# Sleepwalking/libllsm2

Hardware: AMD Instinct MI355X
Metric: frames/sec (layer0 analyze+synth, 44.1 kHz, 5 ms hop) (higher is better)
Workload: dtype f32; 1 GPU; 1024 synthetic 1 s utterances per GPU, F0 120 Hz fixed, 44.1 kHz, 5 ms hop, layer0 analyze+synth, default options, f0_refine=0; utterances_per_gpu=1024, frames_per_utterance=200, parallelism=dp1

## Files before the change

include/llsm_gpu.h:

```cpp
#ifndef LLSM_AMD_LLSM_GPU_H
#define LLSM_AMD_LLSM_GPU_H

#include <stddef.h>
#include "llsm.h"

#ifdef __cplusplus
extern "C" {
#endif

typedef struct llsm_gpu_context llsm_gpu_context;
typedef struct llsm_gpu_batch   llsm_gpu_batch;

int         llsm_gpu_device_count(void);
const char* llsm_gpu_last_error(void);

llsm_gpu_context* llsm_gpu_create_context(int device, void* stream);
void              llsm_gpu_delete_context(llsm_gpu_context* ctx);
void*             llsm_gpu_context_stream(llsm_gpu_context* ctx);
int               llsm_gpu_synchronize(llsm_gpu_context* ctx);

int llsm_gpu_set_convention(const char* name, int value);
int llsm_gpu_get_convention(const char* name);

void llsm_gpu_release_cached_memory(void);
// ... 197 lines not shown
  FP_TYPE* eenv_ampl; FP_TYPE* eenv_phse;
} llsm_flat_params;
int llsm_chunk_to_flat(llsm_chunk* src, llsm_flat_params* dst, int frm_off);
void llsm_slab_stats(long long* live_slabs, long long* live_bytes, long long* pooled_bytes);
void llsm_slab_trim(void);
void llsm_delete_chunks(llsm_chunk** chunks, int n);
void llsm_gpu_release_cached_batches(void);
int llsm_flat_to_chunk(const llsm_flat_params* src, int frm_off, llsm_chunk* dst);

size_t      llsm_chunk_blob_size(llsm_chunk* src);
long long   llsm_chunk_to_blob(llsm_chunk* src, void* dst, size_t capacity);
int         llsm_blob_view(const void* blob, size_t bytes, llsm_flat_params* view, int* nfrm,
  FP_TYPE* thop, FP_TYPE* fnyq);
llsm_chunk* llsm_blob_to_chunk(const void* blob, size_t bytes);
int         llsm_blob_view_l1(const void* blob, size_t bytes, llsm_flat_l1* view);
int         llsm_gpu_batch_upload_blob(llsm_gpu_batch* b, int utt, const void* blob, size_t bytes);
int         llsm_gpu_batch_upload_blobs(llsm_gpu_batch* b, int utt0, int n, const void* const* blobs, const size_t* bytes);
size_t      llsm_blob_bytes(int nfrm, int maxnhar, int maxnhar_e, int npsd, int nchannel, int nchanfreq, int nspec);
int         llsm_gpu_batch_blob_sizes(llsm_gpu_batch* b, int utt0, int n, size_t* sizes);
int         llsm_gpu_batch_download_blobs(llsm_gpu_batch* b, int utt0, int n, void* const* dst, const size_t* capacity);
int         llsm_gpu_batch_download_blob_block(llsm_gpu_batch* b, int utt0, int n, void* block, size_t capacity, size_t* offsets);

typedef void llsm_rtsynth_group;
llsm_rtsynth_group* llsm_create_rtsynth_group(llsm_soptions* options, llsm_container* conf,
  int capacity_samples, int n_streams);
void llsm_delete_rtsynth_group(llsm_rtsynth_group* g);
int  llsm_rtsynth_group_getlatency(llsm_rtsynth_group* g);
int  llsm_rtsynth_group_numoutput(llsm_rtsynth_group* g, int stream);
void llsm_rtsynth_group_feed(llsm_rtsynth_group* g, llsm_container** frames);
void llsm_rtsynth_group_feed_many(llsm_rtsynth_group* g, llsm_container** frames, int n_hops);
int       llsm_gpu_rt_graph(int on);
int       llsm_gpu_shared_f0_tiles(int on);
int       llsm_gpu_synth_tables(int on);
int       llsm_gpu_pbp_real_ifft(int on);
int       llsm_gpu_analysis_overlap(int on);
long long llsm_gpu_rt_graph_hops(void);
int       llsm_gpu_rt_pipeline(int on);
int       llsm_gpu_rt_fused(int on);
int       llsm_gpu_rt_direct(int on);
int  llsm_rtsynth_group_fetch(llsm_rtsynth_group* g, int stream, FP_TYPE* dst_p, FP_TYPE* dst_ap,
  int max_samples);
int  llsm_rtsynth_group_fetch_all(llsm_rtsynth_group* g, FP_TYPE* dst_p, FP_TYPE* dst_ap, int max_samples,
  int* counts);

void llsm_gpu_set_default_seed(unsigned long long seed);

int llsm_gpu_plan_index(int which, int i, int j, FP_TYPE f0, FP_TYPE thop,
  FP_TYPE fs, FP_TYPE rel_winsize);

#ifdef __cplusplus
}
#endif
#endif
```

libllsm2_amd/__init__.py:

```python
import ctypes as C
import os

import numpy as np

_HERE = os.path.dirname(os.path.abspath(__file__))
LIB_PATH = os.environ.get("LLSM_AMD_LIB", os.path.join(_HERE, "libllsm2_amd.so"))

fp = C.c_float
P_fp = C.POINTER(C.c_float)
P_int = C.POINTER(C.c_int)


class Container(C.Structure):
    _fields_ = [("members", C.POINTER(C.c_void_p)), ("destructors", C.POINTER(C.c_void_p)),
                ("copyctors", C.POINTER(C.c_void_p)), ("nmember", C.c_int)]


class HMFrame(C.Structure):
    _fields_ = [("ampl", P_fp), ("phse", P_fp), ("nhar", C.c_int)]


class NMFrame(C.Structure):
    _fields_ = [("eenv", C.POINTER(C.POINTER(HMFrame))), ("edc", P_fp), ("psd", P_fp),
                ("npsd", C.c_int), ("nchannel", C.c_int)]
# ... 81 lines not shown
llsm_create_nmframe llsm_copy_nmframe llsm_copy_nmframe_inplace llsm_delete_nmframe
llsm_create_pbpeffect llsm_copy_pbpeffect llsm_delete_pbpeffect
llsm_create_frame llsm_frame_phaseshift llsm_frame_phasesync_rps llsm_frame_checklayer0
llsm_frame_checklayer1 llsm_conf_checklayer0 llsm_conf_checklayer1 llsm_delete_output
llsm_frame_tolayer0 llsm_chunk_tolayer1 llsm_chunk_tolayer0
llsm_gpu_batch_enable_layer1 llsm_gpu_batch_tolayer1 llsm_gpu_batch_tolayer0 llsm_gpu_batch_set_maxnhar_conf
llsm_gpu_batch_set_pbpeffect llsm_chunk_to_flat_l1 llsm_flat_l1_to_chunk
llsm_refine_f0 llsm_compute_spectrogram llsm_compute_dc llsm_harmonic_peakpicking llsm_harmonic_czt
llsm_harmonic_analysis llsm_subband_energy llsm_fft_to_psd llsm_estimate_psd llsm_warp_frequency
llsm_spectral_mean llsm_spectrum_from_envelope llsm_get_fftsize llsm_synthesize_harmonic_frame
llsm_synthesize_harmonic_frame_iczt llsm_generate_white_noise llsm_generate_bandlimited_noise
llsm_lipfilter llsm_lipfilter_reim llsm_harmonic_spectrum llsm_harmonic_envelope llsm_harmonic_minphase
llsm_create_cached_glottal_model llsm_delete_cached_glottal_model llsm_spectral_glottal_fitting
llsm_smoothing_filter llsm_lfmodel_from_rd llsm_lfmodel_spectrum llsm_lfmodel_to_gfm llsm_gfm_to_lfmodel
llsm_synthesize_harmonic_frame_auto llsm_make_filtered_pulse
llsm_create_coder llsm_delete_coder llsm_coder_encode llsm_coder_decode_layer1 llsm_coder_decode_layer0
llsm_coder_dimension llsm_coder_encode_frames llsm_coder_decode_frames
llsm_create_aoptions llsm_delete_aoptions llsm_aoptions_toconf
llsm_create_soptions llsm_delete_soptions
llsm_create_chunk llsm_copy_chunk llsm_delete_chunk llsm_chunk_phasesync_rps
llsm_chunk_phasepropagate llsm_chunk_getf0 llsm_analyze llsm_synthesize
llsm_create_rtsynth_buffer llsm_delete_rtsynth_buffer llsm_rtsynth_buffer_getlatency
llsm_rtsynth_buffer_numoutput llsm_rtsynth_buffer_feed llsm_rtsynth_buffer_fetch
llsm_rtsynth_buffer_fetch_decomposed llsm_rtsynth_buffer_clear
llsm_gpu_device_count llsm_gpu_last_error llsm_gpu_create_context llsm_gpu_delete_context
llsm_gpu_context_stream llsm_gpu_synchronize llsm_gpu_set_profiling llsm_gpu_profile_only llsm_gpu_reset_profile
llsm_gpu_get_profile llsm_gpu_fft_selftest llsm_gpu_release_cached_memory llsm_gpu_create_batch llsm_gpu_delete_batch llsm_gpu_batch_layout
llsm_gpu_batch_offsets llsm_gpu_alloc_host llsm_gpu_free_host llsm_gpu_batch_upload llsm_gpu_batch_download llsm_gpu_batch_device_ptr
llsm_gpu_batch_array_bytes llsm_gpu_batch_analyze llsm_gpu_batch_synthesize
llsm_analyze_batch llsm_synthesize_batch llsm_chunk_to_flat llsm_flat_to_chunk
llsm_gpu_set_default_seed llsm_gpu_plan_index llsm_gpu_batch_set_fnyq llsm_gpu_batch_debug_plane llsm_gpu_sum_outputs llsm_gpu_set_convention llsm_gpu_get_convention llsm_gpu_set_fanout llsm_fanout_plan llsm_fanout_selftest
llsm_chunk_blob_size llsm_chunk_to_blob llsm_blob_view llsm_blob_to_chunk llsm_blob_view_l1 llsm_gpu_batch_upload_blob llsm_gpu_batch_upload_blobs
llsm_create_rtsynth_group llsm_delete_rtsynth_group llsm_rtsynth_group_getlatency
llsm_rtsynth_group_numoutput llsm_rtsynth_group_feed llsm_rtsynth_group_feed_many llsm_rtsynth_group_fetch llsm_rtsynth_group_fetch_all llsm_gpu_rt_graph llsm_gpu_rt_graph_hops llsm_gpu_rt_fused llsm_gpu_rt_direct llsm_gpu_rt_pipeline llsm_gpu_analysis_overlap llsm_slab_stats llsm_slab_trim llsm_delete_chunks llsm_gpu_release_cached_batches llsm_gpu_device_numa_node llsm_gpu_bind_thread_to_device llsm_gpu_batch_packed_words llsm_gpu_batch_download_packed llsm_gpu_batch_upload_packed llsm_gpu_batch_download_outputs llsm_gpu_batch_download_packed_block llsm_gpu_batch_upload_packed_block llsm_gpu_batch_transfer_many llsm_gpu_batch_params_layout llsm_gpu_batch_transfer_params llsm_gpu_shared_f0_tiles llsm_gpu_synth_tables llsm_gpu_pbp_real_ifft llsm_frame_compute_snr
llsm_gpu_batch_phasesync_rps llsm_gpu_batch_phasepropagate llsm_gpu_batch_retime llsm_gpu_retime_uniform_positions
llsm_gpu_batch_pitch_formant llsm_gpu_batch_splice
llsm_gpu_batch_enable_coder llsm_gpu_batch_coder_dimension llsm_gpu_batch_encode llsm_gpu_batch_decode
llsm_blob_bytes llsm_gpu_batch_blob_sizes llsm_gpu_batch_download_blobs llsm_gpu_batch_download_blob_block
llsm_gpu_f0_default_options llsm_gpu_f0_plan llsm_gpu_batch_estimate_f0
llsm_gpu_f0_track_default_options llsm_gpu_f0_track_check llsm_gpu_batch_track_f0
llsm_gpu_align_default_options llsm_gpu_align_check llsm_gpu_batch_align
llsm_gpu_batch_align_band llsm_gpu_align_band_min llsm_gpu_align_band_rows
llsm_gpu_batch_align_slope llsm_gpu_align_slope_rows
llsm_gpu_batch_align_band_slope llsm_gpu_align_band_slope_min llsm_gpu_align_band_slope_rows
llsm_gpu_select_default_options llsm_gpu_select_check llsm_gpu_batch_select llsm_gpu_batch_select_chain
""".split()

_lib = None


def load():
    global _lib
    if _lib is not None:
        return _lib
    if not os.path.exists(LIB_PATH):
        from . import build as _b
        _b.build()
    L = C.CDLL(LIB_PATH)
    vp = C.c_void_p
    L.llsm_gpu_last_error.restype = C.c_char_p
    L.llsm_gpu_create_context.restype = vp
    L.llsm_gpu_create_context.argtypes = [C.c_int, vp]
    L.llsm_gpu_delete_context.argtypes = [vp]
    L.llsm_gpu_context_stream.restype = vp
    L.llsm_gpu_context_stream.argtypes = [vp]
    L.llsm_gpu_synchronize.argtypes = [vp]
    L.llsm_gpu_set_profiling.argtypes = [vp, C.c_int]
# ... 164 lines not shown
    L.llsm_copy_hmframe.restype = C.POINTER(HMFrame)
    L.llsm_copy_hmframe.argtypes = [C.POINTER(HMFrame)]
    L.llsm_delete_hmframe.argtypes = [C.POINTER(HMFrame)]
    L.llsm_hmframe_phaseshift.argtypes = [C.POINTER(HMFrame), fp]
    L.llsm_create_nmframe.restype = C.POINTER(NMFrame)
    L.llsm_create_nmframe.argtypes = [C.c_int, C.c_int, C.c_int]
    L.llsm_copy_nmframe.restype = C.POINTER(NMFrame)
    L.llsm_copy_nmframe.argtypes = [C.POINTER(NMFrame)]
    L.llsm_delete_nmframe.argtypes = [C.POINTER(NMFrame)]
    L.llsm_create_frame.restype = C.POINTER(Container)
    L.llsm_create_frame.argtypes = [C.c_int, C.c_int, C.c_int, C.c_int]
    L.llsm_frame_checklayer0.argtypes = [C.POINTER(Container)]
    L.llsm_conf_checklayer0.argtypes = [C.POINTER(Container)]
    L.llsm_create_rtsynth_buffer.restype = vp
    L.llsm_create_rtsynth_buffer.argtypes = [C.POINTER(SOptions), C.POINTER(Container), C.c_int]
    L.llsm_delete_rtsynth_buffer.argtypes = [vp]
    L.llsm_rtsynth_buffer_getlatency.argtypes = [vp]
    L.llsm_rtsynth_buffer_numoutput.argtypes = [vp]
    L.llsm_rtsynth_buffer_feed.argtypes = [vp, C.POINTER(Container)]
    L.llsm_rtsynth_buffer_fetch.argtypes = [vp, P_fp]
    L.llsm_rtsynth_buffer_fetch_decomposed.argtypes = [vp, P_fp, P_fp]
    L.llsm_rtsynth_buffer_clear.argtypes = [vp]
    L.llsm_create_rtsynth_group.restype = vp
    L.llsm_create_rtsynth_group.argtypes = [C.POINTER(SOptions), C.POINTER(Container), C.c_int, C.c_int]
    L.llsm_delete_rtsynth_group.argtypes = [vp]
    L.llsm_rtsynth_group_getlatency.argtypes = [vp]
    L.llsm_rtsynth_group_numoutput.argtypes = [vp, C.c_int]
    L.llsm_rtsynth_group_feed.argtypes = [vp, C.POINTER(C.POINTER(Container))]
    L.llsm_rtsynth_group_fetch.argtypes = [vp, C.c_int, P_fp, P_fp, C.c_int]
    L.llsm_rtsynth_group_fetch_all.argtypes = [vp, P_fp, P_fp, C.c_int, P_int]
    L.llsm_gpu_rt_graph.argtypes = [C.c_int]
    L.llsm_gpu_shared_f0_tiles.argtypes = [C.c_int]
    L.llsm_gpu_synth_tables.argtypes = [C.c_int]
    L.llsm_gpu_pbp_real_ifft.argtypes = [C.c_int]
    L.llsm_gpu_rt_fused.argtypes = [C.c_int]
    L.llsm_gpu_rt_direct.argtypes = [C.c_int]
    L.llsm_gpu_rt_pipeline.argtypes = [C.c_int]
    L.llsm_gpu_analysis_overlap.argtypes = [C.c_int]
    L.llsm_gpu_rt_graph_hops.restype = C.c_longlong
    _lib = L
    return L


class LlsmError(RuntimeError):
    pass


def _check(rc, what):
    if rc != 0:
        raise LlsmError(f"{what}: {load().llsm_gpu_last_error().decode()}")


def make_aoptions(**kw):
    o = AOptions()
    o.thop, o.maxnhar, o.maxnhar_e, o.npsd, o.nchannel = 0.005, 100, 4, 256, 4
    o.lip_radius, o.f0_refine, o.hm_method, o.rel_winsize = 1.5, 1, HMCZT, 4.0
    cf = kw.pop("chanfreq", [2000.0, 4000.0, 8000.0])
    for k, v in kw.items():
        setattr(o, k, v)
    o._cf = (fp * max(len(cf), 1))(*cf)
    o.chanfreq = C.cast(o._cf, P_fp)
    return o


def retime_uniform_positions(nfrm_src, nfrm_dst):
    pos = np.zeros(max(int(nfrm_dst), 0), np.float32)
# ... 423 lines not shown
```

libllsm2_amd/csrc/dev_common.h:

```cpp
#pragma once
#include <hip/hip_runtime.h>
#include <stdint.h>
#include "kernels.h"

#define WAVE 64
#define DEV __device__ __forceinline__

DEV float wave_sum(float v) {
#pragma unroll
  for(int o = 32; o > 0; o >>= 1) v += __shfl_xor(v, o, WAVE);
  return v;
}

DEV float wave_max(float v) {
#pragma unroll
  for(int o = 32; o > 0; o >>= 1) v = fmaxf(v, __shfl_xor(v, o, WAVE));
  return v;
}

typedef __amdgpu_buffer_rsrc_t buf_t;
DEV buf_t buf_range(const float* p, int lo, int hi) {
  const int n = hi > lo ? hi - lo : 0;
  return __builtin_amdgcn_make_buffer_rsrc((void*)(p + lo), 0, n * 4, 0x00020000);
}
DEV float ld_range(buf_t r, int idx_minus_lo) {
  int off = idx_minus_lo * 4;
  asm volatile("" : "+v"(off));
  return __builtin_bit_cast(float, __builtin_amdgcn_raw_buffer_load_b32(r, off, 0, 0));
}
DEV float ld_range_b(buf_t r, int byte_off) {
  asm volatile("" : "+v"(byte_off));
  return __builtin_bit_cast(float, __builtin_amdgcn_raw_buffer_load_b32(r, byte_off, 0, 0));
}

DEV void cs_turns(double turns, float* c, float* s) {
  const float y = (float)((turns - rint(turns)) * 4.0);
  const float k = rintf(y);
  const float r = y - k, r2 = r * r;
  float sn = fmaf(r2, 1.6044118478735982e-4f, -4.681754135318688e-3f);
  sn = fmaf(r2, sn, 7.969262624616704e-2f);
  sn = fmaf(r2, sn, -6.459640975062462e-1f);
  sn = fmaf(r2, sn, 1.5707963267948966f) * r;
  float cs = fmaf(r2, -2.5202042373060605e-5f, 9.1926027483942658e-4f);
  cs = fmaf(r2, cs, -2.0863480763352960e-2f);
  cs = fmaf(r2, cs, 2.5366950790104800e-1f);
  cs = fmaf(r2, cs, -1.2337005501361697f);
  cs = fmaf(r2, cs, 1.0f);
  const int q = (int)k & 3;
  const float c1 = (q & 1) ? -sn : cs, s1 = (q & 1) ? cs : sn;
  *c = (q & 2) ? -c1 : c1;
  *s = (q & 2) ? -s1 : s1;
}

DEV void cs_turns_rel(double turns, float* c, float* s) {
  const double y = (turns - rint(turns)) * 4.0;
  const double kd = rint(y);
  const float r = (float)(y - kd), r2 = r * r;
  float sn = fmaf(r2, 1.6044118478735982e-4f, -4.681754135318688e-3f);
  sn = fmaf(r2, sn, 7.969262624616704e-2f);
  sn = fmaf(r2, sn, -6.459640975062462e-1f);
  sn = fmaf(r2, sn, 1.5707963267948966f) * r;
// ... 140 lines not shown
```

libllsm2_amd/csrc/engine.cpp:

```cpp
#include <hip/hip_runtime.h>
#include <sched.h>

#include <algorithm>
#include <atomic>
#include <cctype>
#include <cmath>
#include <cstdio>
#include <cstring>
#include <map>
#include <mutex>
#include <string>
#include <vector>

#include "kernels.h"
#include "cheby.h"
#include "engine.h"
#include "llsm_gpu.h"
#include "plan.h"
#include "batch.h"

namespace lp = llsm_plan;

namespace {
struct HostConventions { int hann_periodic = 0, mavg_half = 3, filtfilt_pad = 15, interp1u_excl = 0, kalman_init = 0, lobe_1e6 = 133979, lf_rd_clamp = 0; } g_hconv;
// ... 271 lines not shown
extern "C" void llsm_gpu_release_cached_memory(void) {
  DevPool& P = pool_here();
  std::vector<void*> drop;
  {
    std::lock_guard<std::mutex> lock(P.m);
    for(auto& kv : P.free_) { drop.push_back(kv.second); P.size_.erase(kv.second); }
    P.free_.clear(); P.cached = 0;
  }
  for(void* q : drop) hipFree(q);
}

static int ilog2(int n) { int l = 0; while((1 << l) < n) l ++; return l; }

static int hann_sym(int n) { return n <= 1 ? 0 : (g_hconv.hann_periodic ? n : n - 1); }
static std::vector<float> make_hann(int n) {
  std::vector<float> w(n);
  const int den = g_hconv.hann_periodic ? n : n - 1;
  for(int i = 0; i < n; i ++)
    w[i] = n == 1 ? 1.0f : (float)(0.5 - 0.5 * std::cos(2.0 * 3.14159265358979323846 * (i <= den - i ? i : den - i) / den));
  return w;
}
static std::vector<float> make_blackman(int n) {
  std::vector<float> w(n);
  for(int i = 0; i < n; i ++) {
    double t = 2.0 * 3.14159265358979323846 * i / (n - 1);
    w[i] = n == 1 ? 1.0f : (float)(0.42 - 0.5 * std::cos(t) + 0.08 * std::cos(2.0 * t));
  }
  return w;
}
static std::atomic<int> g_f0_tiles([] { const char* e = std::getenv("LLSM_GPU_F0_TILES"); return e ? (std::atoi(e) > 0 ? 1 : 0) : 1; }());
extern "C" int llsm_gpu_shared_f0_tiles(int on) { if(on >= 0) g_config_epoch.fetch_add(1); return on < 0 ? g_f0_tiles.load() : g_f0_tiles.exchange(on > 0 ? 1 : 0); }
static std::atomic<int> g_synth_tables([] { const char* e = std::getenv("LLSM_GPU_SYNTH_TABLES"); return e ? (std::atoi(e) > 0 ? 1 : 0) : 1; }());
extern "C" int llsm_gpu_synth_tables(int on) { if(on >= 0) g_config_epoch.fetch_add(1); return on < 0 ? g_synth_tables.load() : g_synth_tables.exchange(on > 0 ? 1 : 0); }

static BatchDev batch_dev(llsm_gpu_batch* b, float fs) {
  BatchDev d;
  d.n_utt = b -> lay.n_utt; d.nframes = b -> lay.total_frames;
  d.maxnhar = b -> lay.maxnhar; d.maxnhar_e = b -> lay.maxnhar_e;
  d.npsd = b -> lay.npsd; d.nchannel = b -> lay.nchannel;
  d.thop = b -> opt.thop; d.fs = fs; d.rel_winsize = b -> opt.rel_winsize;
  d.x_off = b -> d_x_off.p; d.nx = b -> d_nx.p; d.frm_off = b -> d_frm_off.p; d.nfrm = b -> d_nfrm.p;
  d.frm_utt = b -> d_frm_utt.p;
  d.f0 = (float*)b -> arr[LLSM_GPU_F0]; d.nhar = (int*)b -> arr[LLSM_GPU_NHAR];
  d.ampl = (float*)b -> arr[LLSM_GPU_AMPL]; d.phse = (float*)b -> arr[LLSM_GPU_PHSE];
  d.psd = (float*)b -> arr[LLSM_GPU_PSD]; d.psdres = (float*)b -> arr[LLSM_GPU_PSDRES];
  d.has_psdres = (int*)b -> arr[LLSM_GPU_HAS_PSDRES];
  d.edc = (float*)b -> arr[LLSM_GPU_EDC]; d.nhar_e = (int*)b -> arr[LLSM_GPU_NHAR_E];
  d.eenv_ampl = (float*)b -> arr[LLSM_GPU_EENV_AMPL]; d.eenv_phse = (float*)b -> arr[LLSM_GPU_EENV_PHSE];
  d.x = (const float*)b -> arr[LLSM_GPU_X];
  d.pairs = b -> npairs > 0 ? b -> d_pairs.p : nullptr; d.npairs = b -> npairs;
  const bool tiles = g_f0_tiles.load() > 0;
  d.hblocks = tiles && b -> nhblocks > 0 ? b -> d_hblocks.p : nullptr; d.nhblocks = tiles ? b -> nhblocks : 0;
  d.synth_tables = g_synth_tables.load() > 0 ? 1 : 0;
  return d;
}

static int channel_chain(const llsm_gpu_batch* b, float fs, int c, bool* hp0, float* cut0,
  bool* hp1, float* cut1, bool* from_x) {
  int nch = b -> lay.nchannel;
  float fmin = c == 0 ? 0.0f : b -> chanfreq[c - 1];
  float fmax = c == nch - 1 ? (float)(fs / 2.0) : b -> chanfreq[c];
  *from_x = fmin > 6000.0;
  float c1 = fmin / fs, c2 = fmax / fs;
  if(c1 < 0) c1 = 0;
  if(c2 > 0.5f) c2 = 0.5f;
  if(c1 != 0 && c2 < 0.5f) { *hp0 = true; *cut0 = c1; *hp1 = false; *cut1 = c2; return 2; }
  if(c1 == 0) { *hp0 = false; *cut0 = c2; return 1; }
  *hp0 = true; *cut0 = c1; return 1;
}
static const int kParamIds[11] = {LLSM_GPU_F0, LLSM_GPU_NHAR, LLSM_GPU_AMPL, LLSM_GPU_PHSE, LLSM_GPU_PSD, LLSM_GPU_PSDRES, LLSM_GPU_HAS_PSDRES,
                                  LLSM_GPU_EDC, LLSM_GPU_NHAR_E, LLSM_GPU_EENV_AMPL, LLSM_GPU_EENV_PHSE};


extern "C" llsm_gpu_batch* llsm_gpu_create_batch(llsm_gpu_context* ctx,
  const llsm_aoptions* options, FP_TYPE fs, int n_utt, const int* nx, const int* nfrm) {
  if(! ctx || ! options || n_utt < 0 || n_utt > 65535) {
    llsm_set_error("llsm_gpu_create_batch: bad arguments (n_utt must be 0..65535)"); return nullptr;
  }
  if(options -> nchannel < 1 || options -> nchannel > 8 || options -> maxnhar_e > 8 ||
     options -> maxnhar_e < 0 || options -> maxnhar < 1 || options -> npsd < 2) {
    llsm_set_error("unsupported options: need 1<=nchannel<=8, 0<=maxnhar_e<=8, maxnhar>=1, npsd>=2");
    return nullptr;
  }
  if(n_utt > 0 && (! nx || ! nfrm)) { llsm_set_error("llsm_gpu_create_batch: nx / nfrm missing"); return nullptr; }
  for(int u = 0; u < n_utt; u ++) {
    if(nx[u] < 0 || nfrm[u] < 0) {
// ... 1053 lines not shown
```

libllsm2_amd/csrc/kernels.h:

```cpp
#ifndef LLSM_AMD_KERNELS_H
#define LLSM_AMD_KERNELS_H

#if ! defined(LLSM_KBENCH_EXPERIMENTS) && ( \
    defined(KAL_ABL) || defined(NF_ABL) || defined(KAL_BREAK) || defined(IIR_FAKE_L2) || defined(IIR_GEN_EXPERIMENT) || \
    defined(RT2_TIMING) || defined(HT_TABLE_EXPERIMENT) || \
    defined(HT_SEG) || defined(HT_CHUNK) || defined(HT_WPE) || defined(HE_WPE) || defined(IIR_SEG) || defined(IIR_WPE) || \
    defined(KAL_WPE) || defined(KAL_CHUNK) || defined(EXU_Q) || defined(EXU_WPE) || defined(NF_OLA_WPE) || \
    defined(SO4_WAVES) || defined(SO4_WPE) || defined(PBP_NT) || defined(PBP_WIDE_BELOW) || defined(PBP_WPE) || \
    defined(SYN_UNIT_DIV) || defined(NF_UNIT_DIV))
#error "experiment build switches need -DLLSM_KBENCH_EXPERIMENTS (tools/kbench.py --build); the product library is never built with them"
#endif

#include <hip/hip_runtime.h>
#include <stddef.h>
#include "cheby.h"
#include "packed.h"

struct FiltSectionD {
  double b[5];
  double a[5];
  double zi[4];
  double M[6][16];
  double H[IIR_SEG][4];
};
// ... 8 lines not shown
  float* tmp;
  int n;
  int sec0;
  int sec1;
  int square;
  int pad;
  int fused;
  int wlo, whi;
};

struct DevConventions {
  int mavg_half;
  int interp1u_excl;
  int kalman_init;
  float lobe_bias;
  int lf_rd_clamp;
};
int llsm_l1_kernels_set_conventions(const DevConventions& c);
int llsm_kernels_set_conventions(const DevConventions& c);

struct BatchDev {
  int n_utt, nframes;
  int maxnhar, maxnhar_e, npsd, nchannel;
  float thop, fs, rel_winsize;
  const int* x_off; const int* nx; const int* frm_off; const int* nfrm;
  const int* frm_utt;
  float* f0; int* nhar; float* ampl; float* phse;
  float* psd; float* psdres; int* has_psdres; float* edc; int* nhar_e;
  float* eenv_ampl; float* eenv_phse;
  const float* x;
  const int2* pairs; int npairs;
  const int2* hblocks; int nhblocks;
  int synth_tables;
};

#define LLSM_LDS_FFT_MAX 8192
#define LLSM_BIG_FFT_MAX (1 << 17)
#define LLSM_BIG_FFT_GRID 512
static inline int llsm_big_fft_grid(size_t elems_per_wg) {
  const size_t cap = ((size_t)256 << 20) / sizeof(float2) / (elems_per_wg ? elems_per_wg : 1);
  return (int)(cap < 16 ? 16 : (cap > LLSM_BIG_FFT_GRID ? LLSM_BIG_FFT_GRID : cap));
}

struct LaunchCtx {
  hipStream_t stream;
  void (*prof_begin)(void* user, const char* name, hipStream_t stream);
  void (*prof_end)(void* user, hipStream_t stream);
  void* prof_user;
  const float2* tw_big = nullptr; int tw_big_nmax = 0; float2* big_scratch = nullptr; size_t big_scratch_elems = 0;
};

int launch_refine_f0(LaunchCtx* P, const BatchDev& d);
int launch_harm_speech(LaunchCtx* P, const BatchDev& d, float min_f0);
int launch_harm_env(LaunchCtx* P, const BatchDev& d, const float* ce, size_t ce_stride);
int launch_synth_frames(LaunchCtx* P, const BatchDev& d, int nwin, const float* win,
  const float* cyc_shift, float* frames, int lds_harmonics);
int synth_ola_group_units(void);
int synth_ola_unit_div(int nwin, int lds_harmonics);
int launch_synth_ola(LaunchCtx* P, const BatchDev& d, const int4* units, int nunits, int halo,
  int nwin, const float* win, int lds_harmonics, const int* out_off, const int* out_len,
  const float* x, float* out, int mode, float* mix);
int launch_harm_pp_big(LaunchCtx* P, const BatchDev& d, const float* sig, size_t sig_stride, int nsig,
  const int* nfft_u, int maxnhar, float norm_base, int lds_n, int nmax, int* nhar_out, float* ampl, float* phse);
int launch_filtfilt(LaunchCtx* P, const FiltJob* jobs, int njobs, const FiltSectionD* sections);
int launch_wf_selftest(LaunchCtx* P, int logN, const float2* in, float2* out, int count, int inverse);
int launch_spgm_env(LaunchCtx* P, const BatchDev& d, int nwin_psd, int N, int logN,
// ... 206 lines not shown
```

libllsm2_amd/csrc/synth_kernels.hip:

```cpp
#include <hip/hip_runtime.h>
#include <stdint.h>
#include <algorithm>
#include <climits>

#include "kernels.h"
#include "plan.h"

namespace lp = llsm_plan;
#pragma clang fp contract(fast)
#include "dev_common.h"
#include "synth_frame.h"
#include "launch.h"

extern __shared__ __attribute__((aligned(16))) unsigned char g_lds[];

template <int NT>
__global__ __launch_bounds__(WAVE) void k_synth_frames(
  const int* __restrict__ frm_utt, const int* __restrict__ frm_off,
  const float* __restrict__ f0, const int* __restrict__ nhar,
  const float* __restrict__ ampl, const float* __restrict__ phse, int maxnhar,
  float thop, float fs, int nwin, int L, const float* __restrict__ win,
  const float* __restrict__ cyc_shift, float* __restrict__ frames) {
  const int g = blockIdx.x, lane = threadIdx.x;
  const float f = f0[g];
// ... 54 lines not shown
        if(mode == 0) out[oo + s] = xv[k] - rv[k];
        else {
          out[oo + s] = rv[k];
          if(mix) mix[oo + s] = rv[k] + xv[k];
        }
      }
    }
  };
  for(int j = j0; j < i1; j ++) {
    const float f = f0[fo + j];
    if(!(f > 0)) continue;
    const int st = lp::center(j, thop, fs) - nwin / 2;
    advance(st);
    __syncthreads();
    synth_frame<NT>(fo + j, j, f, nhar, ampl, phse, maxnhar, thop, fs, nwin, L, win, nullptr, A, lane,
      [&](int t, float v) { ring[(st + t) & (R - 1)] += v; });
    __syncthreads();
  }
  advance(own_hi);
}

#ifndef SO4_WAVES
#define SO4_WAVES 4
#endif
#ifndef SO4_WPE
#define SO4_WPE 4
#endif
#define SYN_TAB_MAXKS 32
struct So4Args {
  const int4* units; int halo, R;
  const int* frm_off; const int* nfrm; const int* out_off; const int* out_len;
  const float* f0; const int* nhar; const float* ampl; const float* phse; int maxnhar;
  float thop, fs; int nwin, L; const float* win; int lds_harmonics, nks_tab, use_tab;
  const float* x; float* out; int mode; float* mix;
};

__global__ __launch_bounds__(SO4_WAVES * WAVE, SO4_WPE) void k_synth_ola4(const So4Args P) {
  const int lane = threadIdx.x & (WAVE - 1), wv = threadIdx.x >> 6;
  const int R = P.R, nwin = P.nwin, L = P.L, maxnhar = P.maxnhar;
  const float thop = P.thop, fs = P.fs;
  float4* tab = (float4*)g_lds;
  float2* A = (float2*)(tab + (size_t)P.nks_tab * WAVE) + (size_t)wv * (P.lds_harmonics + 4);
  float* ring = (float*)((float2*)(tab + (size_t)P.nks_tab * WAVE) + (size_t)SO4_WAVES * (P.lds_harmonics + 4)) + (size_t)wv * R;
  for(int t = lane; t < R; t += WAVE) ring[t] = 0.0f;
  const int grp = xcd_frame(blockIdx.x, gridDim.x);
  const int4 unit0 = P.units[SO4_WAVES * grp];
  const int4 unit = P.units[SO4_WAVES * grp + wv];
  const int u = unit.x, i0 = unit.y, i1 = unit.z;
  const int nf = P.nfrm[u], fo = P.frm_off[u], len = P.out_len[u];
  const int row = lane & 15, q = lane >> 4;
  float f_tab = 0.0f;
  if(P.use_tab) {
    const int jg = max(0, unit0.y - P.halo);
    const int jj = jg + lane;
    const float fl = jj < nf ? P.f0[P.frm_off[unit0.x] + jj] : 0.0f;
    const unsigned long long vm = __ballot(fl > 0);
    if(vm) f_tab = __shfl(fl, __ffsll((long long)vm) - 1, WAVE);
  }
  if(f_tab > 0 && wv == 0) {
    const double turn1 = (double)f_tab / (double)fs;
    const int rho = L * (row - 8) + L / 2;
    const double ta = turn1 * (double)rho, tb = turn1 * (double)row;
    float u4r, u4i, s4r, s4i;
    cs_turns(4.0 * ta, & u4r, & u4i);
    cs_turns(4.0 * tb, & s4r, & s4i);
    float vr = 1.0f, vi = 0.0f, bx = 1.0f, by = 0.0f;
    for(int ks = 0; ks < P.nks_tab; ks ++) {
      const int h = 4 * ks + q;
      if((ks & (SYN_RESEED - 1)) == 0) {
        cs_turns(ta * (double)(h + 1), & vr, & vi);
        cs_turns(tb * (double)(h + 1), & bx, & by);
      }
      tab[ks * WAVE + lane] = make_float4(vr, vi, bx, by);
      syn_rot(vr, vi, u4r, u4i);
      syn_rot(bx, by, s4r, s4i);
    }
  }
  __syncthreads();
  if(unit.w != 0) return;
  const size_t oo = (size_t)P.out_off[u];
  const int own_lo = i0 == 0 ? 0 : min(max(lp::center(i0, thop, fs) - nwin / 2, 0), len);
  const int own_hi = i1 >= nf ? len : min(max(lp::center(i1, thop, fs) - nwin / 2, 0), len);
  const int j0 = max(0, i0 - P.halo);
  int flushed = lp::center(j0, thop, fs) - nwin / 2;
  const float* xb = (P.x && len > 0) ? P.x + oo : nullptr;
  float* out = P.out; float* mix = P.mix; const int mode = P.mode;
  float xq[4] = {0.0f, 0.0f, 0.0f, 0.0f}; int pf_base = INT_MIN;
  auto prefetch_x = [&](int from) {
    pf_base = from;
    if(! xb) return;
#pragma unroll
    for(int k = 0; k < 4; k ++) xq[k] = xb[min(max(from + lane + WAVE * k, 0), len - 1)];
  };
  auto advance = [&](int target) {
    for(; flushed < target; flushed = min(flushed + 4 * WAVE, target)) {
      float rv[4], xv[4]; bool own[4];
      const bool pre = flushed == pf_base;
#pragma unroll
      for(int k = 0; k < 4; k ++) {
        const int s = flushed + lane + WAVE * k;
        const bool ok = s < target;
        own[k] = ok && s >= own_lo && s < own_hi;
        rv[k] = ring[s & (R - 1)];
        xv[k] = pre ? xq[k] : (xb ? xb[own[k] ? s : 0] : 0.0f);
        if(ok) ring[s & (R - 1)] = 0.0f; else rv[k] = 0.0f;
      }
#pragma unroll
      for(int k = 0; k < 4; k ++) {
        const int s = flushed + lane + WAVE * k;
        if(! own[k]) continue;
        if(mode == 0) out[oo + s] = xv[k] - rv[k];
        else {
          out[oo + s] = rv[k];
          if(mix) mix[oo + s] = rv[k] + xv[k];
        }
      }
    }
  };
  const int half = nwin / 2;
  int tP[4], tM[4]; float wP[4], wM[4];
#pragma unroll
  for(int r = 0; r < 4; r ++) {
    const int tc = L * (4 * q + r - 8) + L / 2 + half;
    const int tp = tc + row, tm = tc - row;
    const bool okp = row < L / 2 && tp >= 0 && tp < nwin;
    const bool okm = row >= 1 && row <= L / 2 && tm >= 0 && tm < nwin;
    tP[r] = okp ? tp : -1; tM[r] = okm ? tm : -1;
    wP[r] = okp ? P.win[tp] : 0.0f; wM[r] = okm ? P.win[tm] : 0.0f;
  }
  const unsigned f_tab_bits = __float_as_uint(f_tab);
  struct Row { float f; int K; float a0, a1, p0, p1; };
  auto load_row = [&](int j) {
    Row r; r.f = 0.0f; r.K = 0; r.a0 = r.a1 = r.p0 = r.p1 = 0.0f;
    if(j < i1) {
      const int g = fo + j;
      r.f = P.f0[g]; r.K = P.nhar[g];
      const float* ar = P.ampl + (size_t)g * maxnhar; const float* pr = P.phse + (size_t)g * maxnhar;
      if(lane < maxnhar) { r.a0 = ar[lane]; r.p0 = pr[lane]; }
      if(lane + WAVE < maxnhar) { r.a1 = ar[lane + WAVE]; r.p1 = pr[lane + WAVE]; }
    }
    return r;
  };
  Row cur = load_row(j0);
  for(int j = j0; j < i1; j ++) {
    const Row rw = cur;
    cur = load_row(j + 1);
    const float f = rw.f;
    if(!(f > 0)) continue;
    const int st = lp::center(j, thop, fs) - nwin / 2;
    advance(st);
    prefetch_x(st);
    int K = rw.K; if(K > 2048) K = 2048; if(K > maxnhar) K = maxnhar; if(K < 0) K = 0;
    const int Kp = (K + 3) & ~3, nks = Kp / 4;
    __builtin_amdgcn_fence(__ATOMIC_RELEASE, "workgroup");
    __builtin_amdgcn_wave_barrier();
    {
      const float corr = syn_corr(j, thop, fs, f);
#pragma unroll
      for(int m = 0; m < 2; m ++) {
        const int k = lane + WAVE * m;
        if(k < Kp) {
          float2 v = make_float2(0.0f, 0.0f);
          if(k < K) {
            const double phd = (double)(m ? rw.p1 : rw.p0) - (double)corr * (k + 1.0);
            float sn, cs; cs_turns(phd * 0.15915494309189533577, & cs, & sn);
            const float a = m ? rw.a1 : rw.a0;
            v = make_float2(a * cs, a * sn);
          }
          A[k] = v;
        }
      }
    }
    __builtin_amdgcn_fence(__ATOMIC_RELEASE, "workgroup");
    __builtin_amdgcn_wave_barrier();
    __builtin_amdgcn_fence(__ATOMIC_ACQUIRE, "workgroup");
    f32x4 accE = (f32x4){0, 0, 0, 0}, accO = (f32x4){0, 0, 0, 0};
    if(__float_as_uint(f) == f_tab_bits && nks <= P.nks_tab) {
      const float4* tl = tab + lane;
      const float2* Aq = A + q;
      int ks = 0;
      for(; ks + 4 <= nks; ks += 4) {
        float2 a[4]; float4 t[4];
#pragma unroll
        for(int m = 0; m < 4; m ++) { a[m] = Aq[4 * (ks + m)]; t[m] = tl[(ks + m) * WAVE]; }
#pragma unroll
        for(int m = 0; m < 4; m ++) {
          accE = __builtin_amdgcn_mfma_f32_16x16x4f32(syn_pr(a[m], t[m].x, t[m].y), t[m].z, accE, 0, 0, 0);
          accO = __builtin_amdgcn_mfma_f32_16x16x4f32(syn_npi(a[m], t[m].x, t[m].y), t[m].w, accO, 0, 0, 0);
        }
      }
      for(; ks < nks; ks ++) {
        const float2 a = Aq[4 * ks]; const float4 t = tl[ks * WAVE];
        accE = __builtin_amdgcn_mfma_f32_16x16x4f32(syn_pr(a, t.x, t.y), t.z, accE, 0, 0, 0);
        accO = __builtin_amdgcn_mfma_f32_16x16x4f32(syn_npi(a, t.x, t.y), t.w, accO, 0, 0, 0);
      }
    } else {
      const double turn1 = (double)f / (double)fs;
      const int rho = L * (row - 8) + L / 2;
      const double ta = turn1 * (double)rho, tb = turn1 * (double)row;
      float u4r, u4i, s4r, s4i;
      cs_turns(4.0 * ta, & u4r, & u4i);
      cs_turns(4.0 * tb, & s4r, & s4i);
      float vr = 1.0f, vi = 0.0f, bx = 1.0f, by = 0.0f;
      for(int ks = 0; ks < nks; ks ++) {
        const int h = 4 * ks + q;
        if((ks & (SYN_RESEED - 1)) == 0) {
          cs_turns(ta * (double)(h + 1), & vr, & vi);
          cs_turns(tb * (double)(h + 1), & bx, & by);
        }
        const float2 a = A[h];
        accE = __builtin_amdgcn_mfma_f32_16x16x4f32(syn_pr(a, vr, vi), bx, accE, 0, 0, 0);
        accO = __builtin_amdgcn_mfma_f32_16x16x4f32(syn_npi(a, vr, vi), by, accO, 0, 0, 0);
        syn_rot(vr, vi, u4r, u4i);
        syn_rot(bx, by, s4r, s4i);
      }
    }
#pragma unroll
    for(int r = 0; r < 4; r ++) {
      const float e = accE[r], o = accO[r];
      if(tP[r] >= 0) ring[(st + tP[r]) & (R - 1)] += (e + o) * wP[r];
      if(tM[r] >= 0) ring[(st + tM[r]) & (R - 1)] += (e - o) * wM[r];
    }
  }
  __builtin_amdgcn_fence(__ATOMIC_RELEASE, "workgroup");
  __builtin_amdgcn_wave_barrier();
  advance(own_hi);
}

static bool synth_ola_uses_groups(int nwin, int lds_harmonics) {
  return synth_tiles(nwin).T == 1 && lds_harmonics <= 4 * SYN_TAB_MAXKS;
}
int synth_ola_unit_div(int nwin, int lds_harmonics) { return synth_ola_uses_groups(nwin, lds_harmonics) ? 4096 : 8192; }
int synth_ola_group_units(void) { return SO4_WAVES; }
int launch_synth_frames(LaunchCtx* P, const BatchDev& d, int nwin, const float* win,
  const float* cyc_shift, float* frames, int lds_harmonics) {
  if(d.nframes == 0) return 0;
  const SynthTiles t = synth_tiles(nwin);
  const size_t lds = (lds_harmonics + 4) * sizeof(float2);
  return with_tiles(t.NT, [&](auto nts) {
    LAUNCH("k_synth_frames", (k_synth_frames<nts>), dim3(d.nframes), dim3(WAVE), lds,
      d.frm_utt, d.frm_off, d.f0, d.nhar, d.ampl, d.phse, d.maxnhar, d.thop, d.fs, nwin, t.L, win, cyc_shift, frames);
    return 0;
  });
}

int launch_synth_ola(LaunchCtx* P, const BatchDev& d, const int4* units, int nunits, int halo,
  int nwin, const float* win, int lds_harmonics, const int* out_off, const int* out_len,
  const float* x, float* out, int mode, float* mix) {
  if(nunits == 0) return 0;
  const SynthTiles t = synth_tiles(nwin);
  int R = 64; while(R < nwin) R <<= 1;
  if(synth_ola_uses_groups(nwin, lds_harmonics) && nunits % SO4_WAVES == 0) {
    So4Args a;
    a.units = units; a.halo = halo; a.R = R; a.frm_off = d.frm_off; a.nfrm = d.nfrm; a.out_off = out_off; a.out_len = out_len;
    a.f0 = d.f0; a.nhar = d.nhar; a.ampl = d.ampl; a.phse = d.phse; a.maxnhar = d.maxnhar; a.thop = d.thop; a.fs = d.fs;
    a.nwin = nwin; a.L = t.L; a.win = win; a.lds_harmonics = lds_harmonics; a.nks_tab = (lds_harmonics + 3) / 4;
    a.use_tab = d.synth_tables; a.x = x; a.out = out; a.mode = mode; a.mix = mix;
    const size_t lds4 = (size_t)a.nks_tab * WAVE * sizeof(float4)
      + SO4_WAVES * ((lds_harmonics + 4) * sizeof(float2) + R * sizeof(float));
    LAUNCH("k_synth_ola4", k_synth_ola4, dim3(nunits / SO4_WAVES), dim3(SO4_WAVES * WAVE), lds4, a);
    return 0;
  }
  const size_t lds = (lds_harmonics + 4) * sizeof(float2) + R * sizeof(float);
  return with_tiles(t.NT, [&](auto nts) {
    LAUNCH("k_synth_ola", (k_synth_ola<nts>), dim3(nunits), dim3(WAVE), lds,
      units, halo, R, d.frm_off, d.nfrm, out_off, out_len, d.f0, d.nhar, d.ampl, d.phse, d.maxnhar,
      d.thop, d.fs, nwin, t.L, win, lds_harmonics, x, out, mode, mix);
    return 0;
  });
}
```

Baseline: 35.93 million frames/s.

## Specialize grouped synth OLA kernel by mode and make flushes branch-free with buffer ops

Templates k_synth_ola4 on output mode and on whether x and mix are present, so the per-sample branches on those pointers disappear. Flush and ring-accumulate paths become branch-free: invalid lanes write to a per-lane dump slot, and global stores go through bounded buffer loads and stores instead of conditionals. The frame-row loads also use buffer ranges. Wave-uniform values are pinned with readfirstlane, and the x prefetch and next-row load move after the LDS table fill to overlap latency. Fences are narrowed to LDS scope, and a runtime toggle for the grouped path is added. The extra LDS per wave and five template instantiations cost a little occupancy and code size.

```diff
diff --git a/include/llsm_gpu.h b/include/llsm_gpu.h
--- a/include/llsm_gpu.h
+++ b/include/llsm_gpu.h
@@ -253,6 +253,7 @@
 int       llsm_gpu_rt_graph(int on);
 int       llsm_gpu_shared_f0_tiles(int on);
 int       llsm_gpu_synth_tables(int on);
+int       llsm_gpu_synth_ola_grouped(int on);
 int       llsm_gpu_pbp_real_ifft(int on);
 int       llsm_gpu_analysis_overlap(int on);
 long long llsm_gpu_rt_graph_hops(void);
diff --git a/libllsm2_amd/__init__.py b/libllsm2_amd/__init__.py
--- a/libllsm2_amd/__init__.py
+++ b/libllsm2_amd/__init__.py
@@ -137,7 +137,7 @@
 llsm_gpu_set_default_seed llsm_gpu_plan_index llsm_gpu_batch_set_fnyq llsm_gpu_batch_debug_plane llsm_gpu_sum_outputs llsm_gpu_set_convention llsm_gpu_get_convention llsm_gpu_set_fanout llsm_fanout_plan llsm_fanout_selftest
 llsm_chunk_blob_size llsm_chunk_to_blob llsm_blob_view llsm_blob_to_chunk llsm_blob_view_l1 llsm_gpu_batch_upload_blob llsm_gpu_batch_upload_blobs
 llsm_create_rtsynth_group llsm_delete_rtsynth_group llsm_rtsynth_group_getlatency
-llsm_rtsynth_group_numoutput llsm_rtsynth_group_feed llsm_rtsynth_group_feed_many llsm_rtsynth_group_fetch llsm_rtsynth_group_fetch_all llsm_gpu_rt_graph llsm_gpu_rt_graph_hops llsm_gpu_rt_fused llsm_gpu_rt_direct llsm_gpu_rt_pipeline llsm_gpu_analysis_overlap llsm_slab_stats llsm_slab_trim llsm_delete_chunks llsm_gpu_release_cached_batches llsm_gpu_device_numa_node llsm_gpu_bind_thread_to_device llsm_gpu_batch_packed_words llsm_gpu_batch_download_packed llsm_gpu_batch_upload_packed llsm_gpu_batch_download_outputs llsm_gpu_batch_download_packed_block llsm_gpu_batch_upload_packed_block llsm_gpu_batch_transfer_many llsm_gpu_batch_params_layout llsm_gpu_batch_transfer_params llsm_gpu_shared_f0_tiles llsm_gpu_synth_tables llsm_gpu_pbp_real_ifft llsm_frame_compute_snr
+llsm_rtsynth_group_numoutput llsm_rtsynth_group_feed llsm_rtsynth_group_feed_many llsm_rtsynth_group_fetch llsm_rtsynth_group_fetch_all llsm_gpu_rt_graph llsm_gpu_rt_graph_hops llsm_gpu_rt_fused llsm_gpu_rt_direct llsm_gpu_rt_pipeline llsm_gpu_analysis_overlap llsm_slab_stats llsm_slab_trim llsm_delete_chunks llsm_gpu_release_cached_batches llsm_gpu_device_numa_node llsm_gpu_bind_thread_to_device llsm_gpu_batch_packed_words llsm_gpu_batch_download_packed llsm_gpu_batch_upload_packed llsm_gpu_batch_download_outputs llsm_gpu_batch_download_packed_block llsm_gpu_batch_upload_packed_block llsm_gpu_batch_transfer_many llsm_gpu_batch_params_layout llsm_gpu_batch_transfer_params llsm_gpu_shared_f0_tiles llsm_gpu_synth_tables llsm_gpu_synth_ola_grouped llsm_gpu_pbp_real_ifft llsm_frame_compute_snr
 llsm_gpu_batch_phasesync_rps llsm_gpu_batch_phasepropagate llsm_gpu_batch_retime llsm_gpu_retime_uniform_positions
 llsm_gpu_batch_pitch_formant llsm_gpu_batch_splice
 llsm_gpu_batch_enable_coder llsm_gpu_batch_coder_dimension llsm_gpu_batch_encode llsm_gpu_batch_decode
@@ -368,6 +368,7 @@
     L.llsm_gpu_rt_graph.argtypes = [C.c_int]
     L.llsm_gpu_shared_f0_tiles.argtypes = [C.c_int]
     L.llsm_gpu_synth_tables.argtypes = [C.c_int]
+    L.llsm_gpu_synth_ola_grouped.argtypes = [C.c_int]
     L.llsm_gpu_pbp_real_ifft.argtypes = [C.c_int]
     L.llsm_gpu_rt_fused.argtypes = [C.c_int]
     L.llsm_gpu_rt_direct.argtypes = [C.c_int]
diff --git a/libllsm2_amd/csrc/dev_common.h b/libllsm2_amd/csrc/dev_common.h
--- a/libllsm2_amd/csrc/dev_common.h
+++ b/libllsm2_amd/csrc/dev_common.h
@@ -27,6 +27,11 @@
   int off = idx_minus_lo * 4;
   asm volatile("" : "+v"(off));
   return __builtin_bit_cast(float, __builtin_amdgcn_raw_buffer_load_b32(r, off, 0, 0));
+}
+DEV void st_range(buf_t r, int idx_minus_lo, float v) {
+  int off = idx_minus_lo * 4;
+  asm volatile("" : "+v"(off));
+  __builtin_amdgcn_raw_buffer_store_b32(__builtin_bit_cast(unsigned, v), r, off, 0, 0);
 }
 DEV float ld_range_b(buf_t r, int byte_off) {
   asm volatile("" : "+v"(byte_off));
diff --git a/libllsm2_amd/csrc/engine.cpp b/libllsm2_amd/csrc/engine.cpp
--- a/libllsm2_amd/csrc/engine.cpp
+++ b/libllsm2_amd/csrc/engine.cpp
@@ -327,6 +327,8 @@
 extern "C" int llsm_gpu_shared_f0_tiles(int on) { if(on >= 0) g_config_epoch.fetch_add(1); return on < 0 ? g_f0_tiles.load() : g_f0_tiles.exchange(on > 0 ? 1 : 0); }
 static std::atomic<int> g_synth_tables([] { const char* e = std::getenv("LLSM_GPU_SYNTH_TABLES"); return e ? (std::atoi(e) > 0 ? 1 : 0) : 1; }());
 extern "C" int llsm_gpu_synth_tables(int on) { if(on >= 0) g_config_epoch.fetch_add(1); return on < 0 ? g_synth_tables.load() : g_synth_tables.exchange(on > 0 ? 1 : 0); }
+static std::atomic<int> g_synth_ola_grouped([] { const char* e = std::getenv("LLSM_GPU_SYNTH_OLA_GROUPED"); return e ? (std::atoi(e) > 0 ? 1 : 0) : 1; }());
+extern "C" int llsm_gpu_synth_ola_grouped(int on) { if(on >= 0) g_config_epoch.fetch_add(1); return on < 0 ? g_synth_ola_grouped.load() : g_synth_ola_grouped.exchange(on > 0 ? 1 : 0); }
 
 static BatchDev batch_dev(llsm_gpu_batch* b, float fs) {
   BatchDev d;
@@ -347,6 +349,7 @@
   const bool tiles = g_f0_tiles.load() > 0;
   d.hblocks = tiles && b -> nhblocks > 0 ? b -> d_hblocks.p : nullptr; d.nhblocks = tiles ? b -> nhblocks : 0;
   d.synth_tables = g_synth_tables.load() > 0 ? 1 : 0;
+  d.synth_ola_grouped = g_synth_ola_grouped.load() > 0 ? 1 : 0;
   return d;
 }
 
diff --git a/libllsm2_amd/csrc/kernels.h b/libllsm2_amd/csrc/kernels.h
--- a/libllsm2_amd/csrc/kernels.h
+++ b/libllsm2_amd/csrc/kernels.h
@@ -64,6 +64,7 @@
   const int2* pairs; int npairs;
   const int2* hblocks; int nhblocks;
   int synth_tables;
+  int synth_ola_grouped;
 };
 
 #define LLSM_LDS_FFT_MAX 8192
diff --git a/libllsm2_amd/csrc/synth_kernels.hip b/libllsm2_amd/csrc/synth_kernels.hip
--- a/libllsm2_amd/csrc/synth_kernels.hip
+++ b/libllsm2_amd/csrc/synth_kernels.hip
@@ -110,17 +110,21 @@
   const int* frm_off; const int* nfrm; const int* out_off; const int* out_len;
   const float* f0; const int* nhar; const float* ampl; const float* phse; int maxnhar;
   float thop, fs; int nwin, L; const float* win; int lds_harmonics, nks_tab, use_tab;
-  const float* x; float* out; int mode; float* mix;
+  const float* x; float* out; float* mix;
 };
-
+DEV int so4_uniform(int v) { return __builtin_amdgcn_readfirstlane(v); }
+DEV float so4_uniform(float v) { return __builtin_bit_cast(float, __builtin_amdgcn_readfirstlane(__builtin_bit_cast(int, v))); }
+
+template <int MODE, bool HAS_X, bool HAS_MIX>
 __global__ __launch_bounds__(SO4_WAVES * WAVE, SO4_WPE) void k_synth_ola4(const So4Args P) {
-  const int lane = threadIdx.x & (WAVE - 1), wv = threadIdx.x >> 6;
+  const int lane = threadIdx.x & (WAVE - 1), wv = so4_uniform((int)(threadIdx.x >> 6));
   const int R = P.R, nwin = P.nwin, L = P.L, maxnhar = P.maxnhar;
   const float thop = P.thop, fs = P.fs;
   float4* tab = (float4*)g_lds;
   float2* A = (float2*)(tab + (size_t)P.nks_tab * WAVE) + (size_t)wv * (P.lds_harmonics + 4);
-  float* ring = (float*)((float2*)(tab + (size_t)P.nks_tab * WAVE) + (size_t)SO4_WAVES * (P.lds_harmonics + 4)) + (size_t)wv * R;
-  for(int t = lane; t < R; t += WAVE) ring[t] = 0.0f;
+  float* ring = (float*)((float2*)(tab + (size_t)P.nks_tab * WAVE) + (size_t)SO4_WAVES * (P.lds_harmonics + 4)) + (size_t)wv * (R + WAVE);
+  const int dump = R + lane;
+  for(int t = lane; t < R + WAVE; t += WAVE) ring[t] = 0.0f;
   const int grp = xcd_frame(blockIdx.x, gridDim.x);
   const int4 unit0 = P.units[SO4_WAVES * grp];
   const int4 unit = P.units[SO4_WAVES * grp + wv];
@@ -157,43 +161,48 @@
   __syncthreads();
   if(unit.w != 0) return;
   const size_t oo = (size_t)P.out_off[u];
-  const int own_lo = i0 == 0 ? 0 : min(max(lp::center(i0, thop, fs) - nwin / 2, 0), len);
-  const int own_hi = i1 >= nf ? len : min(max(lp::center(i1, thop, fs) - nwin / 2, 0), len);
+  const int own_lo = so4_uniform(i0 == 0 ? 0 : min(max(lp::center(i0, thop, fs) - nwin / 2, 0), len));
+  const int own_hi = so4_uniform(i1 >= nf ? len : min(max(lp::center(i1, thop, fs) - nwin / 2, 0), len));
   const int j0 = max(0, i0 - P.halo);
   int flushed = lp::center(j0, thop, fs) - nwin / 2;
-  const float* xb = (P.x && len > 0) ? P.x + oo : nullptr;
-  float* out = P.out; float* mix = P.mix; const int mode = P.mode;
+  const buf_t rx = buf_range((HAS_X ? P.x : P.out) + oo, 0, HAS_X ? len : 0);
+  const buf_t ro = buf_range(P.out + oo, own_lo, own_hi);
+  const buf_t rm = buf_range((HAS_MIX ? P.mix : P.out) + oo, own_lo, HAS_MIX ? own_hi : own_lo);
   float xq[4] = {0.0f, 0.0f, 0.0f, 0.0f}; int pf_base = INT_MIN;
   auto prefetch_x = [&](int from) {
     pf_base = from;
-    if(! xb) return;
-#pragma unroll
-    for(int k = 0; k < 4; k ++) xq[k] = xb[min(max(from + lane + WAVE * k, 0), len - 1)];
+#pragma unroll
+    for(int k = 0; k < 4; k ++) if(HAS_X) xq[k] = ld_range(rx, from + lane + WAVE * k);
+  };
+  const int pass_max = min(4 * WAVE, R), own_n = own_hi - own_lo;
+  auto flush_pass = [&](int target, auto steady) {
+    const int n = min(target - flushed, pass_max);
+    float rv[4], xv[4]; int cell[4], so[4];
+#pragma unroll
+    for(int k = 0; k < 4; k ++) {
+      const int s = flushed + lane + WAVE * k;
+      const bool ok = lane + WAVE * k < n;
+      cell[k] = ok ? (s & (R - 1)) : dump;
+      so[k] = ok && s >= own_lo ? s - own_lo : own_n;
+      xv[k] = ! HAS_X ? 0.0f : decltype(steady)::value ? xq[k] : ld_range(rx, s);
+    }
+#pragma unroll
+    for(int k = 0; k < 4; k ++) rv[k] = ring[cell[k]];
+#pragma unroll
+    for(int k = 0; k < 4; k ++) ring[cell[k]] = 0.0f;
+#pragma unroll
+    for(int k = 0; k < 4; k ++) {
+      if(MODE == 0) st_range(ro, so[k], xv[k] - rv[k]);
+      else {
+        st_range(ro, so[k], rv[k]);
+        if(HAS_MIX) st_range(rm, so[k], rv[k] + xv[k]);
+      }
+    }
+    flushed += n;
   };
   auto advance = [&](int target) {
-    for(; flushed < target; flushed = min(flushed + 4 * WAVE, target)) {
-      float rv[4], xv[4]; bool own[4];
-      const bool pre = flushed == pf_base;
-#pragma unroll
-      for(int k = 0; k < 4; k ++) {
-        const int s = flushed + lane + WAVE * k;
-        const bool ok = s < target;
-        own[k] = ok && s >= own_lo && s < own_hi;
-        rv[k] = ring[s & (R - 1)];
-        xv[k] = pre ? xq[k] : (xb ? xb[own[k] ? s : 0] : 0.0f);
-        if(ok) ring[s & (R - 1)] = 0.0f; else rv[k] = 0.0f;
-      }
-#pragma unroll
-      for(int k = 0; k < 4; k ++) {
-        const int s = flushed + lane + WAVE * k;
-        if(! own[k]) continue;
-        if(mode == 0) out[oo + s] = xv[k] - rv[k];
-        else {
-          out[oo + s] = rv[k];
-          if(mix) mix[oo + s] = rv[k] + xv[k];
-        }
-      }
-    }
+    if(flushed < target && flushed == pf_base) flush_pass(target, std::true_type{});
+    while(flushed < target) flush_pass(target, std::false_type{});
   };
   const int half = nwin / 2;
   int tP[4], tM[4]; float wP[4], wM[4];
@@ -208,29 +217,27 @@
   }
   const unsigned f_tab_bits = __float_as_uint(f_tab);
   struct Row { float f; int K; float a0, a1, p0, p1; };
+  const buf_t rf0 = buf_range(P.f0 + fo, j0, i1), rnh = buf_range((const float*)(P.nhar + fo), j0, i1);
   auto load_row = [&](int j) {
-    Row r; r.f = 0.0f; r.K = 0; r.a0 = r.a1 = r.p0 = r.p1 = 0.0f;
-    if(j < i1) {
-      const int g = fo + j;
-      r.f = P.f0[g]; r.K = P.nhar[g];
-      const float* ar = P.ampl + (size_t)g * maxnhar; const float* pr = P.phse + (size_t)g * maxnhar;
-      if(lane < maxnhar) { r.a0 = ar[lane]; r.p0 = pr[lane]; }
-      if(lane + WAVE < maxnhar) { r.a1 = ar[lane + WAVE]; r.p1 = pr[lane + WAVE]; }
-    }
+    const size_t g = (size_t)(fo + j) * maxnhar;
+    const buf_t ra = buf_range(P.ampl + g, 0, j < i1 ? maxnhar : 0), rp = buf_range(P.phse + g, 0, j < i1 ? maxnhar : 0);
+    Row r;
+    r.a0 = ld_range(ra, lane); r.p0 = ld_range(rp, lane);
+    r.a1 = ld_range(ra, lane + WAVE); r.p1 = ld_range(rp, lane + WAVE);
+    r.K = __builtin_bit_cast(int, ld_range(rnh, j - j0));
+    r.f = ld_range(rf0, j - j0);
     return r;
   };
   Row cur = load_row(j0);
   for(int j = j0; j < i1; j ++) {
     const Row rw = cur;
-    cur = load_row(j + 1);
-    const float f = rw.f;
-    if(!(f > 0)) continue;
+    const float f = so4_uniform(rw.f);
+    if(!(f > 0)) { cur = load_row(j + 1); cur.f = so4_uniform(cur.f); continue; }
     const int st = lp::center(j, thop, fs) - nwin / 2;
     advance(st);
-    prefetch_x(st);
-    int K = rw.K; if(K > 2048) K = 2048; if(K > maxnhar) K = maxnhar; if(K < 0) K = 0;
+    int K = so4_uniform(rw.K); if(K > 2048) K = 2048; if(K > maxnhar) K = maxnhar; if(K < 0) K = 0;
     const int Kp = (K + 3) & ~3, nks = Kp / 4;
-    __builtin_amdgcn_fence(__ATOMIC_RELEASE, "workgroup");
+    __builtin_amdgcn_fence(__ATOMIC_RELEASE, "workgroup", "local");
     __builtin_amdgcn_wave_barrier();
     {
       const float corr = syn_corr(j, thop, fs, f);
@@ -249,9 +256,11 @@
         }
       }
     }
-    __builtin_amdgcn_fence(__ATOMIC_RELEASE, "workgroup");
+    prefetch_x(st);
+    cur = load_row(j + 1);
+    __builtin_amdgcn_fence(__ATOMIC_RELEASE, "workgroup", "local");
     __builtin_amdgcn_wave_barrier();
-    __builtin_amdgcn_fence(__ATOMIC_ACQUIRE, "workgroup");
+    __builtin_amdgcn_fence(__ATOMIC_ACQUIRE, "workgroup", "local");
     f32x4 accE = (f32x4){0, 0, 0, 0}, accO = (f32x4){0, 0, 0, 0};
     if(__float_as_uint(f) == f_tab_bits && nks <= P.nks_tab) {
       const float4* tl = tab + lane;
@@ -293,14 +302,22 @@
         syn_rot(bx, by, s4r, s4i);
       }
     }
+    int cP[4], cM[4]; float rP[4], rM[4];
+#pragma unroll
+    for(int r = 0; r < 4; r ++) {
+      cP[r] = tP[r] >= 0 ? ((st + tP[r]) & (R - 1)) : dump;
+      cM[r] = tM[r] >= 0 ? ((st + tM[r]) & (R - 1)) : dump;
+    }
+#pragma unroll
+    for(int r = 0; r < 4; r ++) { rP[r] = ring[cP[r]]; rM[r] = ring[cM[r]]; }
 #pragma unroll
     for(int r = 0; r < 4; r ++) {
       const float e = accE[r], o = accO[r];
-      if(tP[r] >= 0) ring[(st + tP[r]) & (R - 1)] += (e + o) * wP[r];
-      if(tM[r] >= 0) ring[(st + tM[r]) & (R - 1)] += (e - o) * wM[r];
-    }
-  }
-  __builtin_amdgcn_fence(__ATOMIC_RELEASE, "workgroup");
+      ring[cP[r]] = rP[r] + (e + o) * wP[r];
+      ring[cM[r]] = rM[r] + (e - o) * wM[r];
+    }
+  }
+  __builtin_amdgcn_fence(__ATOMIC_RELEASE, "workgroup", "local");
   __builtin_amdgcn_wave_barrier();
   advance(own_hi);
 }
@@ -322,22 +339,29 @@
   });
 }
 
+template <int MODE, bool HAS_X, bool HAS_MIX>
+static int launch_so4(LaunchCtx* P, const So4Args& a, int groups, size_t lds) {
+  LAUNCH("k_synth_ola4", (k_synth_ola4<MODE, HAS_X, HAS_MIX>), dim3(groups), dim3(SO4_WAVES * WAVE), lds, a);
+  return 0;
+}
 int launch_synth_ola(LaunchCtx* P, const BatchDev& d, const int4* units, int nunits, int halo,
   int nwin, const float* win, int lds_harmonics, const int* out_off, const int* out_len,
   const float* x, float* out, int mode, float* mix) {
   if(nunits == 0) return 0;
   const SynthTiles t = synth_tiles(nwin);
   int R = 64; while(R < nwin) R <<= 1;
-  if(synth_ola_uses_groups(nwin, lds_harmonics) && nunits % SO4_WAVES == 0) {
+  if(d.synth_ola_grouped && synth_ola_uses_groups(nwin, lds_harmonics) && nunits % SO4_WAVES == 0) {
     So4Args a;
     a.units = units; a.halo = halo; a.R = R; a.frm_off = d.frm_off; a.nfrm = d.nfrm; a.out_off = out_off; a.out_len = out_len;
     a.f0 = d.f0; a.nhar = d.nhar; a.ampl = d.ampl; a.phse = d.phse; a.maxnhar = d.maxnhar; a.thop = d.thop; a.fs = d.fs;
     a.nwin = nwin; a.L = t.L; a.win = win; a.lds_harmonics = lds_harmonics; a.nks_tab = (lds_harmonics + 3) / 4;
-    a.use_tab = d.synth_tables; a.x = x; a.out = out; a.mode = mode; a.mix = mix;
+    a.use_tab = d.synth_tables; a.x = x; a.out = out; a.mix = mix;
     const size_t lds4 = (size_t)a.nks_tab * WAVE * sizeof(float4)
-      + SO4_WAVES * ((lds_harmonics + 4) * sizeof(float2) + R * sizeof(float));
-    LAUNCH("k_synth_ola4", k_synth_ola4, dim3(nunits / SO4_WAVES), dim3(SO4_WAVES * WAVE), lds4, a);
-    return 0;
+      + SO4_WAVES * ((lds_harmonics + 4) * sizeof(float2) + (R + WAVE) * sizeof(float));
+    const int groups = nunits / SO4_WAVES;
+    if(mode == 0) return x ? launch_so4<0, true, false>(P, a, groups, lds4) : launch_so4<0, false, false>(P, a, groups, lds4);
+    if(! mix) return launch_so4<1, false, false>(P, a, groups, lds4);
+    return x ? launch_so4<1, true, true>(P, a, groups, lds4) : launch_so4<1, false, true>(P, a, groups, lds4);
   }
   const size_t lds = (lds_harmonics + 4) * sizeof(float2) + R * sizeof(float);
   return with_tiles(t.NT, [&](auto nts) {
```

Result: no change. 36.17 million frames/s (median of 2 runs) (+0.7%).
